# AI4quantum/qiskit-gym

Measured on AMD Instinct MI355X. Metric: env-steps/sec (whole node), CliffordGym 16q x 65536 envs/GPU; bit-exact vs CPU, higher is better.
Workload: dtype u32

## Files before the change

### qiskit_gym_amd/csrc/device_common.hpp

```cpp
#pragma once

#include "qgym_internal.hpp"
#include "qgym_plan.hpp"

namespace qg {

#define QG_WAVE 64

struct KernelClock {
    unsigned long long *slot;
    unsigned long long t0;
    uint32_t waves;
    __device__ inline KernelClock(unsigned long long *s, uint32_t n) : slot(s), t0(wall_clock64()), waves(n) {}
    __device__ inline ~KernelClock() {
        if (slot) {
            asm volatile("s_waitcnt vmcnt(0) lgkmcnt(0)" ::: "memory");
            const unsigned long long t1 = wall_clock64();
            const uint32_t wave = blockIdx.x * ((blockDim.x + 63u) >> 6) + (threadIdx.x >> 6);
            const unsigned long long m = __ballot(1);
            if (wave < waves && __lane_id() == (unsigned)__ffsll((long long)m) - 1u)
                *reinterpret_cast<ulonglong2 *>(slot + 2ull * wave) = make_ulonglong2(t0, t1);
        }
    }
    KernelClock(const KernelClock &) = delete;
    KernelClock &operator=(const KernelClock &) = delete;
};

#ifdef QG_PHASE_CLOCK
__device__ inline void phase_stamp(unsigned long long *slot, uint32_t waves, uint32_t idx) {
    const uint32_t at = 8u * blockIdx.x + idx;
    if (slot && __lane_id() == 0 && idx < 8u && at < waves / 2u) {
        asm volatile("s_waitcnt vmcnt(0) lgkmcnt(0)" ::: "memory");
        const unsigned long long t = wall_clock64();
        *reinterpret_cast<ulonglong2 *>(slot + 2ull * (waves - 1u - at)) = make_ulonglong2(t, t);
    }
}
#else
__device__ inline void phase_stamp(unsigned long long *, uint32_t, uint32_t) {}
#endif

__device__ inline int64_t load_action(const void *actions, uint64_t idx, bool act64) {
    return act64 ? reinterpret_cast<const int64_t *>(actions)[idx]
                 : (int64_t) reinterpret_cast<const int32_t *>(actions)[idx];
}

__device__ inline void done_list_append(uint32_t *list, uint32_t *count, bool fin, uint64_t env, uint64_t cap) {
    const uint64_t m = __ballot(fin);
    if (!m) return;
    const uint32_t lane = __lane_id(), first = (uint32_t)__ffsll((long long)m) - 1u;
    uint32_t base = 0;
    if (lane == first) base = atomicAdd(count, (uint32_t)__popcll(m));
    base = __shfl(base, first);
    const uint32_t slot = base + (uint32_t)__popcll(m & ((1ull << lane) - 1ull));
    if (fin && slot < cap) list[slot] = (uint32_t)env;
}

template <int WAVES = 4>
__device__ inline void done_list_append_block(uint32_t *list, uint32_t *count, bool fin, uint64_t env, uint64_t cap) {
    static_assert(WAVES == 4 || WAVES == 16, "256 or 1 024 threads");
    __shared__ uint32_t wave_count[WAVES], wave_base[WAVES];
    const uint64_t m = __ballot(fin);
    const uint32_t lane = __lane_id(), wave = threadIdx.x >> 6;
    if (lane == 0) wave_count[wave] = (uint32_t)__popcll(m);
    __syncthreads();
    if constexpr (WAVES == 4) {
        if (threadIdx.x == 0) {
            const uint32_t c0 = wave_count[0], c1 = wave_count[1], c2 = wave_count[2], c3 = wave_count[3], total = c0 + c1 + c2 + c3;
            const uint32_t base = total ? atomicAdd(count, total) : 0u;
            wave_base[0] = base;
            wave_base[1] = base + c0;
            wave_base[2] = base + c0 + c1;
// ... 629 lines not shown
```

### qiskit_gym_amd/csrc/kernels_qm.hip

```cpp
#include <cstdlib>

#include "device_common.hpp"
#include "qgym_plan.hpp"
#include "qm_step1.hpp"

namespace qg {


template <int NXP, bool HAS_Z>
struct QmRows {
    static constexpr int R = HAS_Z ? 2 * NXP : NXP;
    static constexpr int G = R / 4;
    static constexpr int xs(int j) { return HAS_Z ? 2 * j : j; }
    static constexpr int zs(int j) { return 2 * j + 1; }
    uint32_t r[R];
};

template <int NXP, bool HAS_Z>
__device__ inline void qm_load(const uint4 *tile, uint32_t lane, QmRows<NXP, HAS_Z> &s) {
#pragma unroll
    for (int g = 0; g < QmRows<NXP, HAS_Z>::G; ++g) {
        const uint4 q = tile[g * 64 + lane];
        s.r[4 * g + 0] = q.x; s.r[4 * g + 1] = q.y; s.r[4 * g + 2] = q.z; s.r[4 * g + 3] = q.w;
    }
// ... 321 lines not shown
                    if (qm_gauss_jordan<NXP, HAS_Z>(s, a.N)) {
                        iflags ^= QM_FLAG_INVERTED;
                        dirty = 0xFFFFFFFFu;
                    } else {
                        fault |= QG_FAULT_SINGULAR;
                    }
                } else {
                    fault |= QG_FAULT_BAD_STATE;
                }
            }
        }
        solved = qm_solved<NXP, HAS_Z>(s, a.N);
        const float achieved = solved ? 1.0f : 0.0f;
        reward = achieved - penalty;
        if (SEQ && a.rewards_seq) a.rewards_seq[(uint64_t)t * a.B + env] = reward;
        if (SEQ && a.dones_seq) a.dones_seq[(uint64_t)t * a.B + env] = (uint8_t)(depth == 0 || solved);
    }

#pragma unroll
    for (int g = 0; g < Rows::G; ++g)
        if ((dirty >> g) & 1u) tile[g * 64 + lane] = make_uint4(s.r[4 * g], s.r[4 * g + 1], s.r[4 * g + 2], s.r[4 * g + 3]);
    a.depth[env] = depth;
    a.reward[env] = reward;
    a.done[env] = (uint8_t)(depth == 0 || solved);
    a.success[env] = (uint8_t)solved;
    if (FEAT && (a.flags & F_TRACK)) {
        a.sol_len[env * 2] = sol_n;
        if (INV) a.sol_len[env * 2 + 1] = sol_b;
    }
    if (INV) a.inverted[env] = (uint8_t)iflags;
    if ((FEAT || INV) && fault) atomicOr(&a.error[env], fault);
    if (a.bad) a.bad[env] = qm_badmask<NXP, HAS_Z>(s, a.N);
}

template <int NXP, bool FEAT, bool LIST = false, bool DENSE = false>
__global__ __launch_bounds__(256) void qm_inv2_kernel(StepArgs a) {
    KernelClock kclk(a.kclk, a.kclk_waves);
    const uint64_t tid = (uint64_t)blockIdx.x * blockDim.x + threadIdx.x;
    __shared__ uint32_t dense_rows[DENSE ? 4 : 1][DENSE ? 32 * 33 : 1];
    uint32_t *dl = DENSE ? dense_rows[threadIdx.x >> 6] : nullptr;
    QG_PREFETCH_STEP_ARGS(a);
    bool whole = false;
    if constexpr (LIST || DENSE) {
        bool fin = false;
        if ((tid >> 1) < a.B) fin = qm_inv2_body<NXP / 2, FEAT, DENSE>(a, NXP / 2, tid >> 1, (uint32_t)tid & 1u, nullptr, dl, &whole);
        if constexpr (DENSE) qm_inv2_dense_flush(a.dense, dl, (tid - (threadIdx.x & 63u)) >> 1, whole);
        if constexpr (LIST) done_mask_store_pairs(a.done_mask, a.B, fin, tid, a.done_epoch);
    } else {
        if ((tid >> 1) >= a.B) return;
        (void)qm_inv2_body<NXP / 2, FEAT, DENSE>(a, NXP / 2, tid >> 1, (uint32_t)tid & 1u, nullptr, dl, &whole);
    }
}

template <int NXP, bool HAS_Z, bool FEAT, bool LIST = false, bool DENSE = false>
__global__ __launch_bounds__(256) void qm_step1_kernel(StepArgs a) {
    KernelClock kclk(a.kclk, a.kclk_waves);
    using Rows = QmRows<NXP, HAS_Z>;
    constexpr int D16 = DENSE ? Rows::R / 16 : 0;
    const uint64_t env = (uint64_t)blockIdx.x * blockDim.x + threadIdx.x;
    QG_PREFETCH_STEP_ARGS(a);
    if constexpr (LIST) {
        bool fin = false;
        if (env < a.B) fin = qm_step1_body<HAS_Z, FEAT, D16>(a, Rows::G, env, load_action(a.actions, env, a.flags & F_ACT64));
        done_mask_store(a.done_mask, a.B, fin, env, a.done_epoch);
    } else {
        if (env >= a.B) return;
        const int64_t act = load_action(a.actions, env, a.flags & F_ACT64);
        (void)qm_step1_body<HAS_Z, FEAT, D16>(a, Rows::G, env, act);
    }
}

template <int NXP, bool HAS_Z, bool ACT64>
__global__ __launch_bounds__(256) void qm_fused_lds_kernel(StepArgs a) {
    using Rows = QmRows<NXP, HAS_Z>;
    __shared__ uint32_t lds_rows[4][Rows::R][QG_WAVE];
    const uint64_t env = (uint64_t)blockIdx.x * blockDim.x + threadIdx.x;
    const uint32_t lane = threadIdx.x & (QG_WAVE - 1);
    if (env >= a.B) return;
    uint32_t (*rows)[QG_WAVE] = lds_rows[threadIdx.x >> 6];
    uint4 *tile = reinterpret_cast<uint4 *>(a.state) + (env >> 6) * (uint64_t)(Rows::G * 64);
    uint32_t bad;
    {
        Rows s;
        qm_load<NXP, HAS_Z>(tile, lane, s);
        bad = qm_badmask<NXP, HAS_Z>(s, a.N);
#pragma unroll
        for (int k = 0; k < Rows::R; ++k) rows[k][lane] = s.r[k];
    }
    int32_t depth = a.depth[env];
    const uint32_t zb = 1u << a.N;
    float reward = 0.0f;
    bool solved = bad == 0;
    auto load_act = [&](uint32_t t) -> int64_t {
        const uint64_t i = (uint64_t)(t < a.T ? t : a.T - 1u) * a.B + env;
        const int64_t v = ACT64 ? reinterpret_cast<const int64_t *>(a.actions)[i] : (int64_t) reinterpret_cast<const int32_t *>(a.actions)[i];
        return t < a.T ? v : -1;
    };
    auto load_gate = [&](int64_t act, GateEntry &g) {
        const bool ok = act >= 0 && act < (int64_t)a.num_actions;
        const GateEntry e = a.gates[ok ? act : 0];
        g.ops = ok ? e.ops : (QM_IDENTITY << 10);
        g.penalty = ok ? e.penalty : 0.0f;
    };
    auto step = [&](uint32_t t, const GateEntry &g) {
        if (t >= a.T) return;
        const uint32_t q0 = g.ops & 31u, q1 = (g.ops >> 5) & 31u, m = (g.ops >> 10) & 0xFFFFu;
        if (m != QM_IDENTITY) {
            const uint32_t sx0 = HAS_Z ? 2u * q0 : q0, sx1 = HAS_Z ? 2u * q1 : q1;
            const uint32_t x0 = rows[sx0][lane], x1 = rows[sx1][lane];
            const uint32_t z0 = HAS_Z ? rows[sx0 + 1u][lane] : 0u, z1 = HAS_Z ? rows[sx1 + 1u][lane] : 0u;
            auto mix = [&](uint32_t k) -> uint32_t {
                const uint32_t b = m >> (4 * k);
                uint32_t o = ((0u - (b & 1u)) & x0) ^ ((0u - ((b >> 2) & 1u)) & x1);
                if (HAS_Z) o ^= ((0u - ((b >> 1) & 1u)) & z0) ^ ((0u - ((b >> 3) & 1u)) & z1);
                return o;
            };
            const uint32_t nx0 = mix(0), nx1 = mix(2), nz0 = HAS_Z ? mix(1) : 0u, nz1 = HAS_Z ? mix(3) : 0u;
            rows[sx1][lane] = nx1;
            if (HAS_Z) rows[sx1 + 1u][lane] = nz1;
            rows[sx0][lane] = nx0;
            if (HAS_Z) rows[sx0 + 1u][lane] = nz0;
            const uint32_t b1 = (uint32_t)(nx1 != (1u << q1) || (HAS_Z && nz1 != (zb << q1)));
            const uint32_t b0 = (uint32_t)(nx0 != (1u << q0) || (HAS_Z && nz0 != (zb << q0)));
// ... 395 lines not shown
#pragma unroll
        for (int sl = 0; sl < Rows::R; ++sl) rows[sl][L] = s.r[sl];
        scramble_flat<uint32_t>(rows, L, a, env);
#pragma unroll
        for (int sl = 0; sl < Rows::R; ++sl) s.r[sl] = rows[sl][L];
    }
    qm_init_finish<NXP, HAS_Z, NO_SET_STATE>(a, env, s);
    if constexpr (!PAIR) after(env, false, false);
}


template <int NXP, bool HAS_Z, int LEAN = 0>
__global__ __launch_bounds__(256) void qm_init_kernel(InitArgs a) {
    KernelClock kclk(a.kclk, a.kclk_waves);
    qm_init_block<NXP, HAS_Z, false, LEAN>(a, blockIdx.x);
}

struct ResetStepArgs {
    InitArgs reset;
    StepArgs step;
    uint32_t reset_blocks;
    uint32_t step_blocks;
    uint32_t first_reset;
};
__device__ inline bool reset_step_role(const ResetStepArgs &ra, uint32_t &index) {
    const uint32_t b = blockIdx.x;
    if (b >= ra.first_reset && b < ra.first_reset + ra.step_blocks) {
        index = b - ra.first_reset;
        return true;
    }
    index = b < ra.first_reset ? b : b - ra.step_blocks;
    return false;
}
template <int NXP, bool HAS_Z, bool FEAT, bool DENSE, bool WAVE = !FEAT>
__global__ __launch_bounds__(256) void qm_reset_step_kernel(ResetStepArgs ra) {
    KernelClock kclk(ra.step.kclk, ra.step.kclk_waves);
    using Rows = QmRows<NXP, HAS_Z>;
    constexpr int D16 = DENSE ? Rows::R / 16 : 0;
    const StepArgs &a = ra.step;
    QG_PREFETCH_STEP_ARGS(a);
    uint32_t role_index;
    if (reset_step_role(ra, role_index)) {
        const uint64_t env = (uint64_t)role_index * blockDim.x + threadIdx.x;
        uint64_t resets = env < a.B ? ra.reset.mask[env >> 6] : 0ull;
        uint32_t relisted = ra.reset.list_count[0];
        relisted = relisted < a.B ? relisted : (uint32_t)a.B;
        for (uint32_t i = 0; i < relisted; ++i) {
            const uint32_t e = ra.reset.list[i];
            if ((e >> 6) == (uint32_t)(env >> 6)) resets |= 1ull << (e & 63u);
        }
        bool fin = false;
        if (env < a.B && !((resets >> (env & 63u)) & 1ull)) {
            const bool alone = D16 != 0 && ((resets >> ((env ^ 1ull) & 63u)) & 1ull);
            fin = qm_step1_body<HAS_Z, FEAT, D16>(a, Rows::G, env, load_action(a.actions, env, a.flags & F_ACT64), alone);
        }
        done_mask_store(a.done_mask, a.B, fin, env, a.done_epoch);
        return;
    }
    qm_init_block<NXP, HAS_Z, false, 1>(ra.reset, role_index, WAVE ? &a : nullptr, [&](uint64_t env, bool stepped, bool fin) {
        if (!stepped) fin = qm_step1_body<HAS_Z, FEAT, D16>(a, Rows::G, env, load_action(a.actions, env, a.flags & F_ACT64), true);
        if (fin) {
            const uint32_t slot = atomicAdd(a.done_count, 1u);
            if (slot < a.B) a.done_list[slot] = (uint32_t)env;
        }
    });
}

template <int NXP, bool FEAT, bool WAVE>
__global__ __launch_bounds__(256) void qm_reset_inv2_step_kernel(ResetStepArgs ra) {
    KernelClock kclk(ra.step.kclk, ra.step.kclk_waves);
    const StepArgs &a = ra.step;
    QG_PREFETCH_STEP_ARGS(a);
    uint32_t role_index;
    if (reset_step_role(ra, role_index)) {
        const uint64_t tid = (uint64_t)role_index * blockDim.x + threadIdx.x, env = tid >> 1;
        uint64_t resets = env < a.B ? ra.reset.mask[env >> 6] : 0ull;
        uint32_t relisted = ra.reset.list_count[0];
        relisted = relisted < a.B ? relisted : (uint32_t)a.B;
        for (uint32_t i = 0; i < relisted; ++i) {
            const uint32_t e = ra.reset.list[i];
            if ((e >> 6) == (uint32_t)(env >> 6)) resets |= 1ull << (e & 63u);
        }
        bool fin = false;
        if (env < a.B && !((resets >> (env & 63u)) & 1ull)) fin = qm_inv2_body<NXP / 2, FEAT, false>(a, NXP / 2, env, (uint32_t)tid & 1u, nullptr);
        done_mask_store_pairs(a.done_mask, a.B, fin, tid, a.done_epoch);
        return;
    }
    const StepArgs *wave_step = WAVE ? &a : nullptr;
    qm_init_block<NXP, true, true, 1>(ra.reset, role_index, wave_step, [&](uint64_t env, uint32_t h, bool stepped, bool fin) {
        if (!stepped) {
            asm volatile("s_waitcnt vmcnt(0)" ::: "memory");
            __builtin_amdgcn_fence(__ATOMIC_ACQUIRE, "agent");
            fin = qm_inv2_body<NXP / 2, FEAT, false>(a, NXP / 2, env, h, nullptr);
        }
        if (fin && h == 0) {
            const uint32_t slot = atomicAdd(a.done_count, 1u);
            if (slot < a.B) a.done_list[slot] = (uint32_t)env;
        }
    });
}

__global__ __launch_bounds__(256) void qm_export_kernel(ObsArgs a, uint32_t nxp, uint32_t has_z) {
    const uint64_t gid = (uint64_t)blockIdx.x * blockDim.x + threadIdx.x;
    const uint64_t env = gid / a.D;
    const uint32_t row = (uint32_t)(gid % a.D);
    if (env >= a.B) return;
    const uint32_t R = has_z ? 2 * nxp : nxp, slot = qm_slot(row, a.N, nxp, has_z);
    const uint32_t *tile = reinterpret_cast<const uint32_t *>(a.state) + (env >> 6) * (uint64_t)(R * 64);
    const uint32_t w = tile[((slot >> 2) * 64 + (uint32_t)(env & 63)) * 4 + (slot & 3)];
    if (a.format == QG_FMT_PACKED) {
        reinterpret_cast<uint32_t *>(a.out)[env * a.out_stride + row] = w;
    } else if (a.format == QG_FMT_I64) {
        int64_t *o = reinterpret_cast<int64_t *>(a.out) + env * a.out_stride + (uint64_t)row * a.D;
// ... 123 lines not shown
            bits |= ((my[pe * PITCH + pr] >> pc) & ((1u << take) - 1u)) << filled;
            filled += take;
            pc = 0;
            if (++pr == D) {
                pr = 0;
                ++pe;
            }
        }
        const uint4 v = expand16_i8(bits);
        if (n_bytes - f >= 16u) {
            *reinterpret_cast<uint4 *>(out + f) = v;
        } else {
            const uint32_t o[4] = {v.x, v.y, v.z, v.w};
            for (uint32_t b = 0; b < n_bytes - f; ++b) out[f + b] = (uint8_t)(o[b >> 2] >> (8u * (b & 3u)));
        }
        c += adv_c;
        if (c >= D) {
            c -= D;
            ++r;
        }
        r += adv_r;
        if (r >= D) {
            r -= D;
            ++e;
        }
        e += adv_e;
    }
}

template <int ES>
__global__ __launch_bounds__(256) void qm_dense_typed_kernel(const uint32_t *state, uint64_t B, uint32_t N, uint32_t D, uint32_t nxp,
                                                             uint32_t has_z, uint32_t chunks_per_row, uint4 *out, uint32_t one) {
    constexpr uint32_t EPC = 16 / ES;
    const uint64_t gid = (uint64_t)blockIdx.x * blockDim.x + threadIdx.x;
    const uint64_t grow = gid / chunks_per_row;
    const uint64_t env = grow / D;
    if (env >= B) return;
    const uint32_t row = (uint32_t)(grow - env * D), c0 = (uint32_t)(gid - grow * chunks_per_row) * EPC;
    const uint32_t R = has_z ? 2 * nxp : nxp, slot = qm_slot(row, N, nxp, has_z);
    const uint32_t *tile = state + (env >> 6) * (uint64_t)(R * 64);
    const uint32_t w = tile[((slot >> 2) * 64 + (uint32_t)(env & 63)) * 4 + (slot & 3)];
    out[gid] = expand_chunk<ES>((w >> c0) & ((1u << EPC) - 1u), one);
}

static inline unsigned grid_for(uint64_t threads, unsigned block) { return (unsigned)((threads + block - 1) / block); }

template <int NXP, bool HAS_Z>
static hipError_t launch_step(const StepArgs &a, hipStream_t s) {
    const dim3 grid(grid_for(a.B, 256)), block(256);
    const bool feat = a.flags & (F_TRACK | F_LAYERS);
    const bool seq = a.T != 1 || a.rewards_seq || a.dones_seq;
    const bool list = a.flags & F_DONE_LIST;
    switch (plan::tile_step(false, plan::tile_inv_kernels(false, HAS_Z, NXP), a.flags, a.T, a.bad != nullptr, a.rewards_seq || a.dones_seq, a.num_actions)) {
    case plan::SK_QM_STEP1: {
        const dim3 lgrid = grid, lblock = block;
        if constexpr (QmRows<NXP, HAS_Z>::R % 16 == 0) {
            if (a.dense) {
                if (feat && list) hipLaunchKernelGGL((qm_step1_kernel<NXP, HAS_Z, true, true, true>), lgrid, lblock, 0, s, a);
                else if (feat) hipLaunchKernelGGL((qm_step1_kernel<NXP, HAS_Z, true, false, true>), grid, block, 0, s, a);
                else if (list) hipLaunchKernelGGL((qm_step1_kernel<NXP, HAS_Z, false, true, true>), lgrid, lblock, 0, s, a);
                else hipLaunchKernelGGL((qm_step1_kernel<NXP, HAS_Z, false, false, true>), grid, block, 0, s, a);
                return hipGetLastError();
            }
        }
        if (feat && list) hipLaunchKernelGGL((qm_step1_kernel<NXP, HAS_Z, true, true>), lgrid, lblock, 0, s, a);
        else if (feat) hipLaunchKernelGGL((qm_step1_kernel<NXP, HAS_Z, true>), grid, block, 0, s, a);
        else if (list) hipLaunchKernelGGL((qm_step1_kernel<NXP, HAS_Z, false, true>), lgrid, lblock, 0, s, a);
        else hipLaunchKernelGGL((qm_step1_kernel<NXP, HAS_Z, false>), grid, block, 0, s, a);
        return hipGetLastError();
    }
    case plan::SK_QM_INV2:
        if constexpr (HAS_Z && NXP <= 16) {
            const dim3 grid2(grid_for(2 * a.B, 256)), lgrid2 = grid2, lblock = block;
            if constexpr (NXP == 16) {
                if (a.dense) {
                    if (feat && list) hipLaunchKernelGGL((qm_inv2_kernel<NXP, true, true, true>), lgrid2, lblock, 0, s, a);
                    else if (feat) hipLaunchKernelGGL((qm_inv2_kernel<NXP, true, false, true>), grid2, block, 0, s, a);
                    else if (list) hipLaunchKernelGGL((qm_inv2_kernel<NXP, false, true, true>), lgrid2, lblock, 0, s, a);
                    else hipLaunchKernelGGL((qm_inv2_kernel<NXP, false, false, true>), grid2, block, 0, s, a);
                    return hipGetLastError();
                }
            }
            if (feat && list) hipLaunchKernelGGL((qm_inv2_kernel<NXP, true, true>), lgrid2, lblock, 0, s, a);
            else if (feat) hipLaunchKernelGGL((qm_inv2_kernel<NXP, true>), grid2, block, 0, s, a);
            else if (list) hipLaunchKernelGGL((qm_inv2_kernel<NXP, false, true>), lgrid2, lblock, 0, s, a);
            else hipLaunchKernelGGL((qm_inv2_kernel<NXP, false>), grid2, block, 0, s, a);
            return hipGetLastError();
        }
        return hipErrorInvalidValue;
    case plan::SK_QM_STEP_GJ:
        if constexpr (HAS_Z && NXP <= 16) {
            hipLaunchKernelGGL((qm_step_kernel<NXP, HAS_Z, true, true, true, true>), grid, block, 0, s, a);
            return hipGetLastError();
        }
        return hipErrorInvalidValue;
    case plan::SK_QM_STEP_INV:
        if constexpr (HAS_Z && NXP <= 16) {
            hipLaunchKernelGGL((qm_step_kernel<NXP, HAS_Z, true, true, true, false>), grid, block, 0, s, a);
            return hipGetLastError();
        }
        return hipErrorInvalidValue;
    case plan::SK_QM_FUSED_LDS:
        if (a.flags & F_ACT64) hipLaunchKernelGGL((qm_fused_lds_kernel<NXP, HAS_Z, true>), grid, block, 0, s, a);
        else hipLaunchKernelGGL((qm_fused_lds_kernel<NXP, HAS_Z, false>), grid, block, 0, s, a);
        return hipGetLastError();
    case plan::SK_QM_STEP:
        if (feat && seq) hipLaunchKernelGGL((qm_step_kernel<NXP, HAS_Z, true, true>), grid, block, 0, s, a);
        else if (feat) hipLaunchKernelGGL((qm_step_kernel<NXP, HAS_Z, true, false>), grid, block, 0, s, a);
        else if (seq) hipLaunchKernelGGL((qm_step_kernel<NXP, HAS_Z, false, true>), grid, block, 0, s, a);
        else hipLaunchKernelGGL((qm_step_kernel<NXP, HAS_Z, false, false>), grid, block, 0, s, a);
        return hipGetLastError();
    default: return hipErrorInvalidValue;
    }
}
template <int NXP, bool HAS_Z>
static hipError_t launch_init(const InitArgs &a, hipStream_t s) {
    const bool lean = a.mode == 2 && a.list;
    uint64_t threads = lean ? 4 * a.B : a.B;
    if (a.list && a.coop && a.n_draws >= 64u) {
        const uint64_t tree_blocks = a.tree_grid;
        if (tree_blocks * QG_TREE_THREADS > threads) threads = tree_blocks * QG_TREE_THREADS;
    }
    if (lean) hipLaunchKernelGGL((qm_init_kernel<NXP, HAS_Z, 1>), dim3(grid_for(threads, 256)), dim3(256), 0, s, a);
// ... 122 lines not shown
```

### qiskit_gym_amd/csrc/qgym_internal.hpp

```cpp
#pragma once

#include <hip/hip_runtime.h>
#include <stdint.h>

#include "../../include/qgym.h"

namespace qg {

struct GateEntry {
    uint32_t ops;
    float penalty;
};
static_assert(sizeof(GateEntry) == 8, "GateEntry must be 8 bytes");

enum : uint32_t { OP_NONE = 0, OP_XOR = 1, OP_SWAP = 2 };
__host__ __device__ inline uint32_t make_op(uint32_t type, uint32_t dst, uint32_t src) {
    return (dst & 63u) | ((src & 63u) << 6) | ((type & 3u) << 12);
}

__host__ __device__ inline uint32_t make_desc(uint32_t kind, uint32_t q0, uint32_t q1) {
    return (kind & 0xFFu) | ((q0 & 0xFFu) << 8) | ((q1 & 0xFFu) << 16);
}

enum : uint32_t {
// ... 106 lines not shown
    uint32_t flags_current;
    uint32_t *nonsymp_flag;
    const uint64_t *clock;
    uint32_t *bad;
    const uint64_t *mask;
    uint32_t mask_words;
    uint32_t mask_epoch;
    uint32_t *count_pub;
    const uint32_t *list;
    uint32_t *list_count;
    uint32_t tree_grid;
    uint32_t *zero_count;
    uint32_t coop;
    const uint32_t *rowops;
    uint64_t env_base;
    uint32_t inverts;
    int8_t *dense;
    unsigned long long *kclk;
    uint32_t kclk_waves;
    uint32_t *count_out;
};

#define QG_CLOCK_SEED_STRIDE 0x9E3779B9ull
__device__ inline uint64_t clock_of(const uint64_t *c) { return c ? *c : 0ull; }
__device__ inline uint64_t step_clock(const StepArgs &a) { return a.step_index + clock_of(a.clock); }
__device__ inline uint64_t init_seed(const InitArgs &a) { return a.seed + QG_CLOCK_SEED_STRIDE * clock_of(a.clock); }

struct ObsArgs {
    const void *state;
    void *out;
    uint64_t B;
    uint64_t out_stride;
    uint32_t D, N, log2L;
    uint32_t format;
    uint32_t obs_rows, obs_cols;
    unsigned long long *kclk;
    uint32_t kclk_waves;
};

#define QG_FMT_BITS 3u
__device__ inline uint64_t bits_window(const uint64_t *bs, uint64_t pos, uint32_t D) {
    const uint32_t sh = (uint32_t)pos & 63u;
    const uint64_t lo = bs[pos >> 6], hi = bs[(pos >> 6) + 1];
    const uint64_t w = sh ? (lo >> sh) | (hi << (64u - sh)) : lo;
    return D >= 64u ? w : w & ((1ull << D) - 1ull);
}

hipError_t lfd_step(const StepArgs &a, bool w64, uint32_t rg, hipStream_t s);
hipError_t lfd_init(const InitArgs &a, bool w64, uint32_t rg, const uint32_t *descs, hipStream_t s);
hipError_t lfd_export(const ObsArgs &a, bool w64, uint32_t rg, const uint8_t *inverted, hipStream_t s);

hipError_t qm_step(const StepArgs &a, uint32_t nxp, bool has_z, hipStream_t s);
hipError_t qm_init(const InitArgs &a, uint32_t nxp, bool has_z, hipStream_t s);
hipError_t qm_reset_step(const InitArgs &reset, const StepArgs &step, uint32_t nxp, bool has_z, hipStream_t s);
hipError_t q64_reset_step(const InitArgs &reset, const StepArgs &step, uint32_t ns, bool has_z, hipStream_t s);
hipError_t qm_export(const ObsArgs &a, uint32_t nxp, bool has_z, hipStream_t s);
hipError_t qm_export_typed(const void *state, uint64_t B, uint32_t N, uint32_t D, uint32_t nxp, bool has_z, void *out, uint32_t elem_size,
                           uint32_t one, hipStream_t s);

hipError_t q64_step(const StepArgs &a, uint32_t ns, bool has_z, hipStream_t s);
hipError_t q64_init(const InitArgs &a, uint32_t ns, bool has_z, hipStream_t s);
hipError_t q64_export(const ObsArgs &a, uint32_t ns, bool has_z, hipStream_t s);

hipError_t lf8_step(const StepArgs &a, bool fused, hipStream_t s);
hipError_t lf8_init(const InitArgs &a, hipStream_t s);
hipError_t lf8_export(const ObsArgs &a, hipStream_t s);

hipError_t word_reset_step(const InitArgs &reset, const StepArgs &step, bool perm, hipStream_t s);
hipError_t perm_step(const StepArgs &a, bool fused, hipStream_t s);
hipError_t perm_init(const InitArgs &a, hipStream_t s);
hipError_t perm_export(const ObsArgs &a, hipStream_t s);
hipError_t permb_step(const StepArgs &a, uint32_t ng, hipStream_t s);
hipError_t permb_init(const InitArgs &a, uint32_t ng, const uint32_t *descs, hipStream_t s);
hipError_t permb_export(const ObsArgs &a, uint32_t ng, hipStream_t s);

hipError_t expand_rows(const void *words_dev, int word_bytes, uint64_t n_rows, uint32_t cols, void *out_dev, int out_dtype, hipStream_t s);
hipError_t expand_rows_i64(const void *words_dev, int word_bytes, uint64_t n_rows, uint32_t cols, int64_t *out_dev, hipStream_t s);
hipError_t pack_bitstream(const void *src, int elem_bytes, uint64_t n_entries, uint64_t *out_words, hipStream_t s);
hipError_t compact_done(const uint8_t *done, uint64_t B, uint32_t *list, uint32_t *count, hipStream_t s);

constexpr uint32_t COPY_MAX_REGIONS = 16;
struct CopyRegionArgs {
    char *dst;
    const char *src;
    uint64_t tile_bytes;
    uint64_t pitch_dst, pitch_src;
    uint32_t rows, w;
};
struct CopyArgs {
    CopyRegionArgs r[COPY_MAX_REGIONS];
    uint32_t n_regions;
    const uint32_t *src_idx;
    const uint32_t *dst_idx;
    uint64_t n, B_src, B_dst;
    int8_t *dense;
    uint32_t D, N, has_z;
};
hipError_t copy_envs(const CopyArgs &a, hipStream_t s);
hipError_t masks_fill(const uint8_t *success, uint8_t *out, uint64_t B, uint32_t num_actions, hipStream_t s);
hipError_t fault_any(const uint32_t *error, uint64_t B, uint32_t *scratch, uint32_t *out_host, hipStream_t s);
hipError_t step_outputs(const float *reward, const uint8_t *done, const uint8_t *success, float *rewards_out, uint8_t *dones_out, uint8_t *success_out,
                        uint64_t B, hipStream_t s);

}
```

### qiskit_gym_amd/csrc/qm_step1.hpp

```cpp
#pragma once

#include "device_common.hpp"

namespace qg {

#define QM_IDENTITY 0x8421u

template <bool HAS_Z>
__device__ inline void qm_group_get(const uint32_t (&u)[4], uint32_t q, uint32_t &x, uint32_t &z) {
    const uint32_t o = 0u - (q & 1u);
    if constexpr (HAS_Z) {
        x = (u[2] & o) | (u[0] & ~o);
        z = (u[3] & o) | (u[1] & ~o);
    } else {
        const uint32_t h = 0u - ((q >> 1) & 1u);
        const uint32_t lo = (u[1] & o) | (u[0] & ~o), hi = (u[3] & o) | (u[2] & ~o);
        x = (hi & h) | (lo & ~h);
        z = 0u;
    }
}
template <bool HAS_Z>
__device__ inline void qm_group_put(uint32_t (&u)[4], uint32_t q, uint32_t x, uint32_t z) {
    if constexpr (HAS_Z) {
        const uint32_t o = 0u - (q & 1u);
        u[0] = (u[0] & o) | (x & ~o); u[1] = (u[1] & o) | (z & ~o);
        u[2] = (x & o) | (u[2] & ~o); u[3] = (z & o) | (u[3] & ~o);
    } else {
#pragma unroll
        for (uint32_t k = 0; k < 4; ++k) u[k] = (q & 3u) == k ? x : u[k];
    }
}

template <bool HAS_Z, bool FEAT, int D16 = 0>
__device__ inline bool qm_step1_body(const StepArgs &a, uint32_t G, uint64_t env, int64_t act, bool alone = false) {
    const uint32_t lane = (uint32_t)env & (QG_WAVE - 1);
    uint4 *tile = reinterpret_cast<uint4 *>(a.state) + (env >> 6) * (uint64_t)(G * 64);
    int32_t depth = a.depth[env];
    const uint32_t bad0 = a.bad[env];
    uint32_t bad = bad0, fault = 0;
    int32_t sol_n = (FEAT && (a.flags & F_TRACK)) ? a.sol_len[env * 2] : 0;
    const bool in_range = act >= 0 && act < (int64_t)a.num_actions;
    float penalty = 0.0f;
    uint32_t drow[4] = {0, 0, 0, 0}, dword[4] = {0, 0, 0, 0}, dchg = 0;
    if (in_range) {
        const GateEntry g = a.gates[act];
        penalty = g.penalty;
        const bool layered = FEAT && (a.flags & F_LAYERS);
        LayerTxn lt;
        if (layered) lt = layers_begin(layer_rec(a.layers, env, 2 * a.N + 2), a.N, a.descs[act]);
        const uint32_t q0 = g.ops & 31u, q1 = (g.ops >> 5) & 31u, m = (g.ops >> 10) & 0xFFFFu;
        if (m != QM_IDENTITY) {
            constexpr uint32_t gsh = HAS_Z ? 1u : 2u;
            const uint32_t g0 = q0 >> gsh, g1 = q1 >> gsh;
            const uint4 va = tile[g0 * 64 + lane], vb = tile[g1 * 64 + lane];
            uint32_t ua[4] = {va.x, va.y, va.z, va.w}, ub[4] = {vb.x, vb.y, vb.z, vb.w};
            uint32_t x0, z0, x1, z1;
            qm_group_get<HAS_Z>(ua, q0, x0, z0);
            qm_group_get<HAS_Z>(ub, q1, x1, z1);
            auto mix = [&](uint32_t k) -> uint32_t {
                const uint32_t b = m >> (4 * k);
                uint32_t o = ((0u - (b & 1u)) & x0) ^ ((0u - ((b >> 2) & 1u)) & x1);
                if (HAS_Z) o ^= ((0u - ((b >> 1) & 1u)) & z0) ^ ((0u - ((b >> 3) & 1u)) & z1);
                return o;
            };
            const uint32_t nx0 = mix(0), nx1 = mix(2), nz0 = HAS_Z ? mix(1) : 0u, nz1 = HAS_Z ? mix(3) : 0u;
            qm_group_put<HAS_Z>(ub, q1, nx1, nz1);
            const bool same = g0 == g1;
#pragma unroll
            for (int k = 0; k < 4; ++k) ua[k] = same ? ub[k] : ua[k];
            qm_group_put<HAS_Z>(ua, q0, nx0, nz0);
            if (!same) tile[g1 * 64 + lane] = make_uint4(ub[0], ub[1], ub[2], ub[3]);
            tile[g0 * 64 + lane] = make_uint4(ua[0], ua[1], ua[2], ua[3]);
            if constexpr (D16 > 0) {
                drow[0] = q0; dword[0] = nx0; dchg |= (uint32_t)(nx0 != x0);
                drow[1] = a.N + q0; dword[1] = nz0; dchg |= (uint32_t)(HAS_Z && nz0 != z0) << 1;
                drow[2] = q1; dword[2] = nx1; dchg |= (uint32_t)(q1 != q0 && nx1 != x1) << 2;
                drow[3] = a.N + q1; dword[3] = nz1; dchg |= (uint32_t)(HAS_Z && q1 != q0 && nz1 != z1) << 3;
            }
            const uint32_t zb = 1u << a.N;
            const uint32_t b1 = (uint32_t)(nx1 != (1u << q1) || (HAS_Z && nz1 != (zb << q1)));
            const uint32_t b0 = (uint32_t)(nx0 != (1u << q0) || (HAS_Z && nz0 != (zb << q0)));
            bad = (bad & ~(1u << q1)) | (b1 << q1);
            bad = (bad & ~(1u << q0)) | (b0 << q0);
        }
        if (layered) penalty = layers_commit(lt, a.w);
    }
    if constexpr (D16 == 2) {
        const bool solo = alone || (env ^ 1ull) >= a.B;
#pragma unroll
        for (int k = 0; k < 4; ++k) {
            if (solo && ((dchg >> k) & 1u)) dense_row_store<2>(a.dense, env, drow[k], dword[k]);
            const uint32_t mine = (!solo && ((dchg >> k) & 1u)) ? (drow[k] | 0x80000000u) : 0u;
#pragma unroll
            for (int par = 0; par < 2; ++par) {
                const uint32_t r = par ? (uint32_t)__builtin_amdgcn_update_dpp(0, (int)mine, 0xF5, 0xF, 0xF, false)
                                       : (uint32_t)__builtin_amdgcn_update_dpp(0, (int)mine, 0xA0, 0xF, 0xF, false);
                const uint32_t w = par ? (uint32_t)__builtin_amdgcn_update_dpp(0, (int)dword[k], 0xF5, 0xF, 0xF, false)
                                       : (uint32_t)__builtin_amdgcn_update_dpp(0, (int)dword[k], 0xA0, 0xF, 0xF, false);
                const uint64_t e = (env & ~1ull) | (uint64_t)par;
                const uint32_t half = lane & 1u;
                if (r >> 31) *reinterpret_cast<uint4 *>(a.dense + (e * 32u + (r & 31u)) * 32u + 16u * half) = expand16_i8(w >> (16u * half));
            }
        }
    } else if constexpr (D16 == 1) {
#pragma unroll
        for (int k = 0; k < 4; ++k)
            if ((dchg >> k) & 1u) dense_row_store<1>(a.dense, env, drow[k], dword[k]);
    }
    if (FEAT && (a.flags & F_TRACK)) {
        if ((uint32_t)sol_n < a.sol_cap) sol_at(a, env, (uint32_t)sol_n++) = sol_word_framed(act, false);
        else fault |= 8u;
    }
    depth = depth > 0 ? depth - 1 : 0;
    const bool solved = bad == 0;
    const float achieved = solved ? 1.0f : 0.0f;
    const float reward = achieved - penalty;
    if (a.rewards_seq) a.rewards_seq[env] = reward;
    if (a.dones_seq) a.dones_seq[env] = (uint8_t)(depth == 0 || solved);
    if (bad != bad0) a.bad[env] = bad;
    a.depth[env] = depth;
    a.reward[env] = reward;
    a.done[env] = (uint8_t)(depth == 0 || solved);
    a.success[env] = (uint8_t)solved;
    if (FEAT && (a.flags & F_TRACK)) a.sol_len[env * 2] = sol_n;
    if (FEAT && fault) atomicOr(&a.error[env], fault);
    return depth == 0 || solved;
}


__device__ inline void qm_inv2_dense_flush(int8_t *dense, const uint32_t *dense_lds, uint64_t env0, bool whole) {
    const uint32_t lane = threadIdx.x & (QG_WAVE - 1);
    __builtin_amdgcn_fence(__ATOMIC_RELEASE, "wavefront");
    __builtin_amdgcn_wave_barrier();
    uint64_t todo = __ballot(whole && !(lane & 1u));
    while (todo) {
        const uint32_t sl = ((uint32_t)__ffsll((long long)todo) - 1u) >> 1;
        todo &= todo - 1ull;
        const uint32_t w = dense_lds[sl * 33u + (lane >> 1)];
        reinterpret_cast<uint4 *>(dense + (env0 + sl) * 1024u)[lane] = expand16_i8(w >> (16u * (lane & 1u)));
    }
}

#define QM_FLAG_INVERTED 1u
#define QM_FLAG_SYMPLECTIC 2u

template <int n>
__device__ inline uint32_t tree_select(const uint32_t (&t)[n], uint32_t q) {
    if constexpr (n == 1) {
        return t[0];
    } else {
        constexpr int m = (n + 1) / 2;
        uint32_t u[m];
        const uint32_t mb = 0u - (q & 1u);
#pragma unroll
        for (int k = 0; k < m; ++k) u[k] = (2 * k + 1 < n) ? ((t[2 * k + 1] & mb) | (t[2 * k] & ~mb)) : t[2 * k];
        return tree_select<m>(u, q >> 1);
    }
}

__device__ inline uint32_t qm_pair_swap(uint32_t v) {
    return (uint32_t)__builtin_amdgcn_update_dpp(0, (int)v, 0xB1, 0xF, 0xF, false);
}

template <int GS, bool FEAT, bool DENSE = false>
__device__ inline bool qm_inv2_body(const StepArgs &a, uint32_t groups, uint64_t env, uint32_t h, const int64_t *act_in, uint32_t *dense_lds = nullptr,
                                    bool *dense_whole = nullptr) {
    const int G = GS ? GS : (int)groups;
    const uint32_t N = a.N;
    uint4 *tile = reinterpret_cast<uint4 *>(a.state) + (env >> 6) * (uint64_t)(G * 64) + (env & 63u);
    uint4 grp[4];
#pragma unroll
    for (int k = 0; k < 4; ++k) {
        grp[k] = make_uint4(0u, 0u, 0u, 0u);
        if (k < G && (h == 0 || k + 4 < G)) grp[k] = tile[(uint32_t)(4 * h + k) * 64u];
    }
    int32_t depth = a.depth[env];
    uint32_t iflags = a.inverted[env];
    uint32_t coin = a.coins ? a.coins[env] : 0u;
    int32_t sol_n = (FEAT && (a.flags & F_TRACK)) ? a.sol_len[env * 2] : 0;
// ... 163 lines not shown
```

Baseline: 21.10 billion.

## Split step1 kernel into own file with scalar args and reordered front loads

Moves the single-step kernel to its own translation unit and passes hot pointers and sizes as direct kernel arguments rather than reading them through the args struct. It also issues the action, depth and bad loads together ahead of a scheduling barrier, makes the gate lookup unconditional (index clamped to 0), and fixes the block size at compile time so the env index needs no blockDim read. The goal is to cut kernel-argument load latency and serialized dependent loads at kernel start. It adds complexity and ablation macros, and the unconditional gate load can read gate 0 for out-of-range actions.

Result: faster. 23.29 billion, median of 6 (+10.4%).

```diff
diff --git a/qiskit_gym_amd/csrc/device_common.hpp b/qiskit_gym_amd/csrc/device_common.hpp
--- a/qiskit_gym_amd/csrc/device_common.hpp
+++ b/qiskit_gym_amd/csrc/device_common.hpp
@@ -10,13 +10,13 @@
 struct KernelClock {
     unsigned long long *slot;
     unsigned long long t0;
-    uint32_t waves;
-    __device__ inline KernelClock(unsigned long long *s, uint32_t n) : slot(s), t0(wall_clock64()), waves(n) {}
+    uint32_t waves, block;
+    __device__ inline KernelClock(unsigned long long *s, uint32_t n, uint32_t block_threads = 0) : slot(s), t0(wall_clock64()), waves(n), block(block_threads) {}
     __device__ inline ~KernelClock() {
         if (slot) {
             asm volatile("s_waitcnt vmcnt(0) lgkmcnt(0)" ::: "memory");
             const unsigned long long t1 = wall_clock64();
-            const uint32_t wave = blockIdx.x * ((blockDim.x + 63u) >> 6) + (threadIdx.x >> 6);
+            const uint32_t wave = blockIdx.x * (((block ? block : blockDim.x) + 63u) >> 6) + (threadIdx.x >> 6);
             const unsigned long long m = __ballot(1);
             if (wave < waves && __lane_id() == (unsigned)__ffsll((long long)m) - 1u)
                 *reinterpret_cast<ulonglong2 *>(slot + 2ull * wave) = make_ulonglong2(t0, t1);
diff --git a/qiskit_gym_amd/csrc/kernels_qm.hip b/qiskit_gym_amd/csrc/kernels_qm.hip
--- a/qiskit_gym_amd/csrc/kernels_qm.hip
+++ b/qiskit_gym_amd/csrc/kernels_qm.hip
@@ -397,23 +397,6 @@
     }
 }
 
-template <int NXP, bool HAS_Z, bool FEAT, bool LIST = false, bool DENSE = false>
-__global__ __launch_bounds__(256) void qm_step1_kernel(StepArgs a) {
-    KernelClock kclk(a.kclk, a.kclk_waves);
-    using Rows = QmRows<NXP, HAS_Z>;
-    constexpr int D16 = DENSE ? Rows::R / 16 : 0;
-    const uint64_t env = (uint64_t)blockIdx.x * blockDim.x + threadIdx.x;
-    QG_PREFETCH_STEP_ARGS(a);
-    if constexpr (LIST) {
-        bool fin = false;
-        if (env < a.B) fin = qm_step1_body<HAS_Z, FEAT, D16>(a, Rows::G, env, load_action(a.actions, env, a.flags & F_ACT64));
-        done_mask_store(a.done_mask, a.B, fin, env, a.done_epoch);
-    } else {
-        if (env >= a.B) return;
-        const int64_t act = load_action(a.actions, env, a.flags & F_ACT64);
-        (void)qm_step1_body<HAS_Z, FEAT, D16>(a, Rows::G, env, act);
-    }
-}
 
 template <int NXP, bool HAS_Z, bool ACT64>
 __global__ __launch_bounds__(256) void qm_fused_lds_kernel(StepArgs a) {
@@ -915,13 +898,13 @@
         bool fin = false;
         if (env < a.B && !((resets >> (env & 63u)) & 1ull)) {
             const bool alone = D16 != 0 && ((resets >> ((env ^ 1ull) & 63u)) & 1ull);
-            fin = qm_step1_body<HAS_Z, FEAT, D16>(a, Rows::G, env, load_action(a.actions, env, a.flags & F_ACT64), alone);
+            fin = qm_step1_body<HAS_Z, FEAT, D16>(step1_front(a), a, Rows::G, env, nullptr, alone);
         }
         done_mask_store(a.done_mask, a.B, fin, env, a.done_epoch);
         return;
     }
     qm_init_block<NXP, HAS_Z, false, 1>(ra.reset, role_index, WAVE ? &a : nullptr, [&](uint64_t env, bool stepped, bool fin) {
-        if (!stepped) fin = qm_step1_body<HAS_Z, FEAT, D16>(a, Rows::G, env, load_action(a.actions, env, a.flags & F_ACT64), true);
+        if (!stepped) fin = qm_step1_body<HAS_Z, FEAT, D16>(step1_front(a), a, Rows::G, env, nullptr, true);
         if (fin) {
             const uint32_t slot = atomicAdd(a.done_count, 1u);
             if (slot < a.B) a.done_list[slot] = (uint32_t)env;
@@ -1151,23 +1134,7 @@
     const bool seq = a.T != 1 || a.rewards_seq || a.dones_seq;
     const bool list = a.flags & F_DONE_LIST;
     switch (plan::tile_step(false, plan::tile_inv_kernels(false, HAS_Z, NXP), a.flags, a.T, a.bad != nullptr, a.rewards_seq || a.dones_seq, a.num_actions)) {
-    case plan::SK_QM_STEP1: {
-        const dim3 lgrid = grid, lblock = block;
-        if constexpr (QmRows<NXP, HAS_Z>::R % 16 == 0) {
-            if (a.dense) {
-                if (feat && list) hipLaunchKernelGGL((qm_step1_kernel<NXP, HAS_Z, true, true, true>), lgrid, lblock, 0, s, a);
-                else if (feat) hipLaunchKernelGGL((qm_step1_kernel<NXP, HAS_Z, true, false, true>), grid, block, 0, s, a);
-                else if (list) hipLaunchKernelGGL((qm_step1_kernel<NXP, HAS_Z, false, true, true>), lgrid, lblock, 0, s, a);
-                else hipLaunchKernelGGL((qm_step1_kernel<NXP, HAS_Z, false, false, true>), grid, block, 0, s, a);
-                return hipGetLastError();
-            }
-        }
-        if (feat && list) hipLaunchKernelGGL((qm_step1_kernel<NXP, HAS_Z, true, true>), lgrid, lblock, 0, s, a);
-        else if (feat) hipLaunchKernelGGL((qm_step1_kernel<NXP, HAS_Z, true>), grid, block, 0, s, a);
-        else if (list) hipLaunchKernelGGL((qm_step1_kernel<NXP, HAS_Z, false, true>), lgrid, lblock, 0, s, a);
-        else hipLaunchKernelGGL((qm_step1_kernel<NXP, HAS_Z, false>), grid, block, 0, s, a);
-        return hipGetLastError();
-    }
+    case plan::SK_QM_STEP1: return qm_step1(a, NXP, HAS_Z, s);
     case plan::SK_QM_INV2:
         if constexpr (HAS_Z && NXP <= 16) {
             const dim3 grid2(grid_for(2 * a.B, 256)), lgrid2 = grid2, lblock = block;
diff --git a/qiskit_gym_amd/csrc/kernels_qm_step1.hip b/qiskit_gym_amd/csrc/kernels_qm_step1.hip
--- /dev/null
+++ b/qiskit_gym_amd/csrc/kernels_qm_step1.hip
@@ -0,0 +1,82 @@
+#include "device_common.hpp"
+#include "qgym_plan.hpp"
+#include "qm_step1.hpp"
+
+namespace qg {
+
+constexpr uint32_t QM_STEP1_BLOCK = 256;
+
+template <int NXP, bool HAS_Z, bool FEAT, bool LIST = false, bool DENSE = false>
+__global__ __launch_bounds__(QM_STEP1_BLOCK) void qm_step1_kernel(const void *actions, int32_t *depth, uint32_t *bad, const GateEntry *gates, void *state,
+                                                                   uint64_t B, uint32_t flags, uint32_t num_actions, StepArgs a) {
+#if QG_STEP1_ABLATE & 4
+    const uint32_t block = blockDim.x;
+    KernelClock kclk(a.kclk, a.kclk_waves);
+#else
+    constexpr uint32_t block = QM_STEP1_BLOCK;
+    KernelClock kclk(a.kclk, a.kclk_waves, QM_STEP1_BLOCK);
+#endif
+    constexpr int R = HAS_Z ? 2 * NXP : NXP, G = R / 4;
+    constexpr int D16 = DENSE ? R / 16 : 0;
+    const Step1Front f{actions, depth, bad, gates, state, B, flags, num_actions};
+    const uint64_t env = (uint64_t)blockIdx.x * block + threadIdx.x;
+    if constexpr (LIST) {
+        bool fin = false;
+        if (env < B) fin = qm_step1_body<HAS_Z, FEAT, D16>(f, a, G, env, nullptr);
+        done_mask_store(a.done_mask, B, fin, env, a.done_epoch);
+    } else {
+        if (env >= B) return;
+        (void)qm_step1_body<HAS_Z, FEAT, D16>(f, a, G, env, nullptr);
+    }
+}
+
+template <int NXP, bool HAS_Z>
+static hipError_t launch_step1(const StepArgs &a, hipStream_t s) {
+    const dim3 grid((unsigned)((a.B + QM_STEP1_BLOCK - 1) / QM_STEP1_BLOCK)), block(QM_STEP1_BLOCK);
+    const bool feat = a.flags & (F_TRACK | F_LAYERS);
+    const bool list = a.flags & F_DONE_LIST;
+#define QM_STEP1_LAUNCH(...) \
+    hipLaunchKernelGGL((qm_step1_kernel<NXP, HAS_Z, __VA_ARGS__>), grid, block, 0, s, a.actions, a.depth, a.bad, a.gates, a.state, a.B, a.flags, a.num_actions, a)
+    constexpr int R = HAS_Z ? 2 * NXP : NXP;
+    if constexpr (R % 16 == 0) {
+        if (a.dense) {
+            if (feat && list) QM_STEP1_LAUNCH(true, true, true);
+            else if (feat) QM_STEP1_LAUNCH(true, false, true);
+            else if (list) QM_STEP1_LAUNCH(false, true, true);
+            else QM_STEP1_LAUNCH(false, false, true);
+            return hipGetLastError();
+        }
+    }
+    if (feat && list) QM_STEP1_LAUNCH(true, true);
+    else if (feat) QM_STEP1_LAUNCH(true);
+    else if (list) QM_STEP1_LAUNCH(false, true);
+    else QM_STEP1_LAUNCH(false);
+#undef QM_STEP1_LAUNCH
+    return hipGetLastError();
+}
+
+hipError_t qm_step1(const StepArgs &a, uint32_t nxp, bool has_z, hipStream_t s) {
+    if (!a.B) return hipSuccess;
+    if (has_z) {
+        switch (nxp) {
+        case 4: return launch_step1<4, true>(a, s);
+        case 8: return launch_step1<8, true>(a, s);
+        case 12: return launch_step1<12, true>(a, s);
+        case 16: return launch_step1<16, true>(a, s);
+        }
+    } else {
+        switch (nxp) {
+        case 4: return launch_step1<4, false>(a, s);
+        case 8: return launch_step1<8, false>(a, s);
+        case 12: return launch_step1<12, false>(a, s);
+        case 16: return launch_step1<16, false>(a, s);
+        case 20: return launch_step1<20, false>(a, s);
+        case 24: return launch_step1<24, false>(a, s);
+        case 28: return launch_step1<28, false>(a, s);
+        case 32: return launch_step1<32, false>(a, s);
+        }
+    }
+    return hipErrorInvalidValue;
+}
+
+}
diff --git a/qiskit_gym_amd/csrc/qgym_internal.hpp b/qiskit_gym_amd/csrc/qgym_internal.hpp
--- a/qiskit_gym_amd/csrc/qgym_internal.hpp
+++ b/qiskit_gym_amd/csrc/qgym_internal.hpp
@@ -182,6 +182,7 @@
 
 hipError_t qm_step(const StepArgs &a, uint32_t nxp, bool has_z, hipStream_t s);
 hipError_t qm_init(const InitArgs &a, uint32_t nxp, bool has_z, hipStream_t s);
+hipError_t qm_step1(const StepArgs &a, uint32_t nxp, bool has_z, hipStream_t s);
 hipError_t qm_reset_step(const InitArgs &reset, const StepArgs &step, uint32_t nxp, bool has_z, hipStream_t s);
 hipError_t q64_reset_step(const InitArgs &reset, const StepArgs &step, uint32_t ns, bool has_z, hipStream_t s);
 hipError_t qm_export(const ObsArgs &a, uint32_t nxp, bool has_z, hipStream_t s);
diff --git a/qiskit_gym_amd/csrc/qm_step1.hpp b/qiskit_gym_amd/csrc/qm_step1.hpp
--- a/qiskit_gym_amd/csrc/qm_step1.hpp
+++ b/qiskit_gym_amd/csrc/qm_step1.hpp
@@ -31,21 +31,83 @@
     }
 }
 
-template <bool HAS_Z, bool FEAT, int D16 = 0>
-__device__ inline bool qm_step1_body(const StepArgs &a, uint32_t G, uint64_t env, int64_t act, bool alone = false) {
+struct Step1Front {
+    const void *actions;
+    int32_t *depth;
+    uint32_t *bad;
+    const GateEntry *gates;
+    void *state;
+    uint64_t B;
+    uint32_t flags, num_actions;
+};
+__device__ inline Step1Front step1_front(const StepArgs &a) { return Step1Front{a.actions, a.depth, a.bad, a.gates, a.state, a.B, a.flags, a.num_actions}; }
+
+#ifndef QG_STEP1_ABLATE
+#define QG_STEP1_ABLATE 0
+#endif
+
+__device__ inline void action_issue(const void *actions, uint64_t idx, bool act64, int32_t &lo, int32_t &hi) {
+    hi = 0;
+    if (act64) {
+        const int64_t v = reinterpret_cast<const int64_t *>(actions)[idx];
+        lo = (int32_t)v;
+        hi = (int32_t)(v >> 32);
+    } else {
+        lo = reinterpret_cast<const int32_t *>(actions)[idx];
+    }
+}
+__device__ inline int64_t action_value(int32_t lo, int32_t hi, bool act64) {
+    hi = act64 ? hi : lo >> 31;
+    return (int64_t)(((uint64_t)(uint32_t)hi << 32) | (uint64_t)(uint32_t)lo);
+}
+
+template <bool HAS_Z, bool FEAT, int D16 = 0, bool PLAIN_FRONT = false>
+__device__ inline bool qm_step1_body(const Step1Front &f, const StepArgs &a, uint32_t G, uint64_t env, const int64_t *act_in, bool alone = false) {
     const uint32_t lane = (uint32_t)env & (QG_WAVE - 1);
-    uint4 *tile = reinterpret_cast<uint4 *>(a.state) + (env >> 6) * (uint64_t)(G * 64);
-    int32_t depth = a.depth[env];
-    const uint32_t bad0 = a.bad[env];
+    uint4 *tile = reinterpret_cast<uint4 *>(f.state) + (env >> 6) * (uint64_t)(G * 64);
+    int64_t act;
+    int32_t depth, sol_n;
+    uint32_t bad0;
+    bool in_range;
+    GateEntry g = GateEntry{QM_IDENTITY << 10, 0.0f};
+    if constexpr (PLAIN_FRONT) {
+        act = act_in ? *act_in : load_action(f.actions, env, f.flags & F_ACT64);
+        depth = f.depth[env];
+        bad0 = f.bad[env];
+        sol_n = (FEAT && (f.flags & F_TRACK)) ? a.sol_len[env * 2] : 0;
+        in_range = act >= 0 && act < (int64_t)f.num_actions;
+        if (in_range) g = f.gates[act];
+    } else {
+        int32_t act_lo = 0, act_hi = 0;
+        if (!act_in) action_issue(f.actions, env, f.flags & F_ACT64, act_lo, act_hi);
+#if QG_STEP1_ABLATE & 1
+        act = act_in ? *act_in : action_value(act_lo, act_hi, f.flags & F_ACT64);
+        __builtin_amdgcn_sched_barrier(0);
+#endif
+        depth = f.depth[env];
+        bad0 = f.bad[env];
+        sol_n = (FEAT && (f.flags & F_TRACK)) ? a.sol_len[env * 2] : 0;
+#if QG_STEP1_ABLATE & 1
+        asm volatile("" : "+v"(bad0));
+        in_range = (uint64_t)act < (uint64_t)f.num_actions;
+        if (in_range) g = f.gates[act];
+#else
+        __builtin_amdgcn_sched_barrier(0);
+        act = act_in ? *act_in : action_value(act_lo, act_hi, f.flags & F_ACT64);
+        in_range = (uint64_t)act < (uint64_t)f.num_actions;
+        const GateEntry entry = f.gates[in_range ? act : 0];
+        if (in_range) g = entry;
+#endif
+        asm volatile("" : "+v"(g.ops), "+v"(g.penalty), "+v"(depth), "+v"(bad0)
+                     : "s"(a.N), "s"(a.rewards_seq), "s"(a.dones_seq), "s"(a.reward), "s"(a.done), "s"(a.success));
+        depth = depth > 0 ? depth - 1 : 0;
+    }
     uint32_t bad = bad0, fault = 0;
-    int32_t sol_n = (FEAT && (a.flags & F_TRACK)) ? a.sol_len[env * 2] : 0;
-    const bool in_range = act >= 0 && act < (int64_t)a.num_actions;
     float penalty = 0.0f;
     uint32_t drow[4] = {0, 0, 0, 0}, dword[4] = {0, 0, 0, 0}, dchg = 0;
     if (in_range) {
-        const GateEntry g = a.gates[act];
         penalty = g.penalty;
-        const bool layered = FEAT && (a.flags & F_LAYERS);
+        const bool layered = FEAT && (f.flags & F_LAYERS);
         LayerTxn lt;
         if (layered) lt = layers_begin(layer_rec(a.layers, env, 2 * a.N + 2), a.N, a.descs[act]);
         const uint32_t q0 = g.ops & 31u, q1 = (g.ops >> 5) & 31u, m = (g.ops >> 10) & 0xFFFFu;
@@ -86,7 +148,7 @@
         if (layered) penalty = layers_commit(lt, a.w);
     }
     if constexpr (D16 == 2) {
-        const bool solo = alone || (env ^ 1ull) >= a.B;
+        const bool solo = alone || (env ^ 1ull) >= f.B;
 #pragma unroll
         for (int k = 0; k < 4; ++k) {
             if (solo && ((dchg >> k) & 1u)) dense_row_store<2>(a.dense, env, drow[k], dword[k]);
@@ -107,24 +169,31 @@
         for (int k = 0; k < 4; ++k)
             if ((dchg >> k) & 1u) dense_row_store<1>(a.dense, env, drow[k], dword[k]);
     }
-    if (FEAT && (a.flags & F_TRACK)) {
+    if (FEAT && (f.flags & F_TRACK)) {
         if ((uint32_t)sol_n < a.sol_cap) sol_at(a, env, (uint32_t)sol_n++) = sol_word_framed(act, false);
         else fault |= 8u;
     }
-    depth = depth > 0 ? depth - 1 : 0;
+#if QG_STEP1_ABLATE & 2
+    if constexpr (!PLAIN_FRONT) asm volatile("s_waitcnt vmcnt(0)" ::: "memory");
+#endif
+    if constexpr (PLAIN_FRONT) depth = depth > 0 ? depth - 1 : 0;
     const bool solved = bad == 0;
     const float achieved = solved ? 1.0f : 0.0f;
     const float reward = achieved - penalty;
     if (a.rewards_seq) a.rewards_seq[env] = reward;
     if (a.dones_seq) a.dones_seq[env] = (uint8_t)(depth == 0 || solved);
-    if (bad != bad0) a.bad[env] = bad;
-    a.depth[env] = depth;
+    if (bad != bad0) f.bad[env] = bad;
+    f.depth[env] = depth;
     a.reward[env] = reward;
     a.done[env] = (uint8_t)(depth == 0 || solved);
     a.success[env] = (uint8_t)solved;
-    if (FEAT && (a.flags & F_TRACK)) a.sol_len[env * 2] = sol_n;
+    if (FEAT && (f.flags & F_TRACK)) a.sol_len[env * 2] = sol_n;
     if (FEAT && fault) atomicOr(&a.error[env], fault);
     return depth == 0 || solved;
+}
+template <bool HAS_Z, bool FEAT, int D16 = 0>
+__device__ inline bool qm_step1_body(const StepArgs &a, uint32_t G, uint64_t env, int64_t act, bool alone = false) {
+    return qm_step1_body<HAS_Z, FEAT, D16, true>(step1_front(a), a, G, env, &act, alone);
 }
 
 
```
